# christoskokas/gtsam-vSLAM

Measured on AMD Instinct MI355X. Metric: frames/sec (extract+match+localBA), 1500 feat stereo 752x480, higher is better.
Workload: dtype u8/i32 (extract, match) + f64 (pose LM, local BA)

## Files before the change

gtsam-vslam_amd/csrc/extract_kernels.hpp:

```cpp
#pragma once
#include "common.hpp"

namespace vslam {

struct PyrDesc {
    int nLevels;
    int w[MAX_LEVELS], h[MAX_LEVELS], pitch[MAX_LEVELS];
    uint32_t off[MAX_LEVELS];
    uint32_t imgStride;
};

struct FastDesc {
    int minXY;
    int edge3;
    int nCols[MAX_LEVELS], nRows[MAX_LEVELS], gridW[MAX_LEVELS], gridH[MAX_LEVELS];
    int cellBase[MAX_LEVELS + 1];
    int cellCap;
    int tileRows, tilePitch;
};

struct BlurDesc {
    int tilesX[MAX_LEVELS];
    int tileBase[MAX_LEVELS + 1];
    int taps[7];
};

struct LevelTables {
    float scalePyr[MAX_LEVELS];
    int scaledPatch[MAX_LEVELS];
};

__host__ __device__ static inline uint32_t pack_cand(int x, int y, int s) {
    return ((uint32_t)y << 20) | ((uint32_t)x << 8) | (uint32_t)s;
}
__host__ __device__ static inline int cand_x(uint32_t p) { return (p >> 8) & 0xfff; }
__host__ __device__ static inline int cand_y(uint32_t p) { return p >> 20; }
__host__ __device__ static inline int cand_s(uint32_t p) { return p & 0xff; }

constexpr int FAST_TILE_PITCH = 80;
constexpr int FAST_TILE_MAX = 76;
constexpr int BLUR_RPT = 16;
constexpr int BLUR_TW = 256, BLUR_TH = 4 * BLUR_RPT;

void launch_load_images(hipStream_t s, const uint8_t* const* dSrc, int stride, uint8_t* pyr, const PyrDesc& P, int nimg);
void launch_load_images_color(hipStream_t s, const uint8_t* const* dSrc, int stride, int channels, uint8_t* pyr, const PyrDesc& P,
                              int nimg);
struct RectSrc {
    const uint8_t* src; const float* mapX; const float* mapY;
    int sw, sh, stride, pad;
};
void launch_load_images_rect(hipStream_t s, const RectSrc* dTab, int channels, uint8_t* pyr, const PyrDesc& P, int nimg);
void launch_resize(hipStream_t s, uint8_t* pyr, const PyrDesc& P, int level, const int2* xtab,
                   const int2* ytab, int nimg);
void launch_fast(hipStream_t s, const uint8_t* pyr, const PyrDesc& P, const FastDesc& F,
                 uint32_t* cellSlots, int* cellCount, int maxThr, int minThr, int nimg);
#ifdef VSLAM_FAST_CHECK
int fast_check_failures(hipStream_t s);
#endif
void launch_gather(hipStream_t s, const uint32_t* cellSlots, const int* cellCount, const FastDesc& F,
                   int nLevels, int* cellOff, uint32_t* cand, int candCap, int* levelCount, int nimg);
void launch_blur(hipStream_t s, const uint8_t* pyr, uint8_t* blur, const PyrDesc& P,
                 const BlurDesc& B, int nimg);
struct DiscRows { int umax[16]; };
void launch_orient_desc(hipStream_t s, const uint8_t* pyr, const uint8_t* blur, const PyrDesc& P,
                        const LevelTables& T, const uint32_t* kept, const int* keptOff, int keptCap,
                        const DiscRows& disc, vslam_keypoint* kps, uint8_t* desc, int outCap,
                        int maxKept, int nimg);
void upload_pattern();

constexpr int SSC_NMAX_LDS = 16384;
constexpr int SSC_NMAX = 65535;
constexpr int SSC_PICKW_G = 2048;
constexpr int SSC_NMAX_MID = 8704;
constexpr int SSC_NMAX_SMALL = 6144;
constexpr int SSC_NMAX_TINY = 3072;
__host__ __device__ static inline int ssc_class(int n, int forceGlobal, int classes = 3) {
    if (forceGlobal || n > SSC_NMAX_LDS) return 1;
    if (n > ((classes & 1) ? SSC_NMAX_MID : SSC_NMAX_SMALL)) return 0;
    if (n > SSC_NMAX_SMALL) return 3;
    return ((classes & 2) && n <= SSC_NMAX_TINY) ? 4 : 2;
}
struct SscArgs {
    const uint32_t* cand; int candCap; const int* levelCount;
    int nLevels, nimg;
    int numRet[MAX_LEVELS], cols[MAX_LEVELS], rows[MAX_LEVELS], high[MAX_LEVELS], kmin[MAX_LEVELS], kmax[MAX_LEVELS];
    uint32_t* tmp;
    uint32_t* gridG;
    const size_t* gridOff;
    uint32_t* aG; uint32_t* sortedG; uint32_t* picksG;
    int forceGlobal;
    int classes;
    int* taskCount;
    int* flags;
};

void launch_ssc(hipStream_t s, const SscArgs& A, uint32_t* kept, int keptCap, int* keptOff, int* hostCounts);

}
```

gtsam-vslam_amd/csrc/ssc.hip:

```cpp
#include "extract_kernels.hpp"
#include <mutex>

namespace vslam {

constexpr int SSC_NT = 512, SSC_NW = SSC_NT / 64;
constexpr int SSC_NPROBE = 8;
constexpr int SSC_COOP_MIN = 2048;
constexpr int SSC_ARENA_WORDS = 20 * 1024;
constexpr int SSC_LONGMAX = 64;

template <int M> struct SscCfg;
template <> struct SscCfg<0> { static constexpr int NMAX = SSC_NMAX_LDS, SEGMAX = 1088, PICKW = SSC_NMAX_LDS / 32, ARENA = SSC_ARENA_WORDS; };
template <> struct SscCfg<1> { static constexpr int NMAX = SSC_NMAX, SEGMAX = 4096, PICKW = SSC_PICKW_G, ARENA = SSC_ARENA_WORDS; };
template <> struct SscCfg<2> { static constexpr int NMAX = SSC_NMAX_SMALL, SEGMAX = 1088, PICKW = SSC_NMAX_SMALL / 32, ARENA = 10 * 1024; };
template <> struct SscCfg<3> { static constexpr int NMAX = SSC_NMAX_MID, SEGMAX = 576, PICKW = SSC_NMAX_MID / 32, ARENA = 10 * 1024; };
template <> struct SscCfg<4> { static constexpr int NMAX = SSC_NMAX_TINY, SEGMAX = 256, PICKW = SSC_NMAX_TINY / 32, ARENA = 4 * 1024; };
template <int M> constexpr int ssc_seg_words() { return 4 * SscCfg<M>::SEGMAX > SSC_NW * 256 ? 4 * SscCfg<M>::SEGMAX : SSC_NW * 256; }
template <int M> constexpr size_t ssc_lds_bytes() {
    return M == 1 ? ((size_t)4 * SscCfg<M>::SEGMAX + (size_t)SscCfg<M>::ARENA) * 4 : ((size_t)2 * SscCfg<M>::NMAX + (size_t)ssc_seg_words<M>()) * 4;
}
template <int M> struct SscCheck {
    using C = SscCfg<M>;
    static_assert(C::SEGMAX - SSC_LONGMAX >= C::NMAX / 17, "every short segment of a tree level needs a list entry");
    static_assert(C::PICKW * 32 >= ((C::NMAX + 63) & ~63), "a probe's pick words cover whole 64-candidate steps");
    static_assert(C::ARENA % SSC_NPROBE == 0 && (M == 1 || C::ARENA / SSC_NPROBE > C::PICKW), "a probing wave's slice holds its pick words and a grid");
    static_assert(M == 1 || C::NMAX + ssc_seg_words<M>() >= C::ARENA, "arena must fit a | seg");
    static constexpr bool ok = true;
};
static_assert(SscCheck<0>::ok && SscCheck<1>::ok && SscCheck<2>::ok && SscCheck<3>::ok && SscCheck<4>::ok, "k_ssc classes");

template <bool G> __device__ __forceinline__ void ssc_fence() {
    if (G) asm volatile("s_waitcnt vmcnt(0) lgkmcnt(0)" ::: "memory");
    else asm volatile("s_waitcnt lgkmcnt(0)" ::: "memory");
}
__device__ __forceinline__ void ssc_lds_fence() { asm volatile("s_waitcnt lgkmcnt(0)" ::: "memory"); }

__device__ __forceinline__ int ssc_cell(int v, int width, float rcpw) {
    const int t = 2 * v;
    int q = (int)((float)t * rcpw);
    q -= (q * width > t);
    q += ((q + 1) * width <= t);
    return q;
}

template <bool G>
__device__ __forceinline__ int ssc_eval(const uint32_t* sc, int n, int width, int cols, int rows, uint32_t* grid, int gridWords,
                                        uint32_t* picks, bool& fits, int abortAbove) {
    const int lane = threadIdx.x & 63;
    const float rcpw = 1.0f / (float)width;
    const int gc = ssc_cell(cols, width, rcpw), gr = ssc_cell(rows, width, rcpw);
    const int span = 2;
    const int rowWords = (gc + 1 + 31) >> 5;
    const int words = (gr + 1) * rowWords;
    fits = words <= gridWords;
    if (!fits) return -1;
    for (int i = lane; i < words; i += 64) grid[i] = 0;
    ssc_lds_fence();
    asm volatile("s_waitcnt vmcnt(0)" ::: "memory");
    int count = 0;
    uint32_t pkNext = lane < n ? sc[lane] : 0u;
    for (int base = 0; base < n; base += 64) {
        const int i = base + lane;
        const bool valid = i < n;
        const uint32_t pk = pkNext;
        if (G) pkNext = (i + 64 < n) ? sc[i + 64] : 0u;
        const int row = ssc_cell(cand_y(pk), width, rcpw);
        const int col = ssc_cell(cand_x(pk), width, rcpw);
        bool covered = true;
        if (valid) covered = (grid[row * rowWords + (col >> 5)] >> (col & 31)) & 1u;
        unsigned long long pend = __ballot(!covered), picked = 0ull;
        while (pend) {
            const int l = __ffsll((long long)pend) - 1;
            picked |= 1ull << l;
            const int rl = __builtin_amdgcn_readlane(row, l), cl = __builtin_amdgcn_readlane(col, l);
            const bool conflict = abs(row - rl) <= span && abs(col - cl) <= span;
            pend &= ~__ballot(conflict);
        }
        if ((picked >> lane) & 1ull) {
            const int r0 = max(row - span, 0), r1 = min(row + span, gr);
            const int c0 = max(col - span, 0), c1 = min(col + span, gc);
            const int w0 = c0 >> 5, w1 = c1 >> 5;
            for (int rr = r0; rr <= r1; rr++) {
                if (w0 == w1) {
                    const uint32_t m = ((1u << (c1 - c0 + 1)) - 1u) << (c0 & 31);
                    atomicOr(&grid[rr * rowWords + w0], m);
                } else {
                    atomicOr(&grid[rr * rowWords + w0], 0xffffffffu << (c0 & 31));
                    atomicOr(&grid[rr * rowWords + w1], 0xffffffffu >> (31 - (c1 & 31)));
                }
            }
        }
        if (picks && lane < 2) picks[(base >> 5) + lane] = (uint32_t)(picked >> (32 * lane));
        count += __popcll(picked);
        if (!G) pkNext = (i + 64 < n) ? sc[i + 64] : 0u;
        ssc_lds_fence();
        asm volatile("s_waitcnt vmcnt(0)" ::: "memory");
        if (abortAbove >= 0 && count > abortAbove) break;
    }
    return count;
}

__device__ int g_sscCoopMin = SSC_COOP_MIN;
__device__ __forceinline__ void ssc_push(uint32_t* segN, int* cntN, int segMax, int f, int e, int depth, int* sFail) {
    if (e - f > g_sscCoopMin) {
        const int q = atomicAdd(cntN + 2, 1);
        if (q < SSC_LONGMAX) { segN[2 * q] = (uint32_t)f | ((uint32_t)e << 16); segN[2 * q + 1] = (uint32_t)depth; }
        else *sFail = 4;
        return;
    }
    const int q = atomicAdd(cntN, 1) + SSC_LONGMAX;
    if (q < segMax) { segN[2 * q] = (uint32_t)f | ((uint32_t)e << 16); segN[2 * q + 1] = (uint32_t)depth; }
    else *sFail = 4;
}

template <bool G>
__device__ void ssc_adjust_heap(uint32_t* first, int holeIndex, int len, uint32_t value) {
    const int topIndex = holeIndex;
    int secondChild = holeIndex;
    while (secondChild < (len - 1) / 2) {
        secondChild = 2 * (secondChild + 1);
        if ((first[secondChild] >> 16) < (first[secondChild - 1] >> 16)) secondChild--;
        first[holeIndex] = first[secondChild];
        ssc_fence<G>();
        holeIndex = secondChild;
    }
    if ((len & 1) == 0 && secondChild == (len - 2) / 2) {
        secondChild = 2 * (secondChild + 1);
        first[holeIndex] = first[secondChild - 1];
        ssc_fence<G>();
        holeIndex = secondChild - 1;
    }
    int parent = (holeIndex - 1) / 2;
    while (holeIndex > topIndex && (first[parent] >> 16) < (value >> 16)) {
        first[holeIndex] = first[parent];
        ssc_fence<G>();
        holeIndex = parent;
        parent = (holeIndex - 1) / 2;
    }
    first[holeIndex] = value;
    ssc_fence<G>();
}
template <bool G>
__device__ void ssc_heapsort(uint32_t* first, int len) {
    if (len < 2) return;
    for (int parent = (len - 2) / 2;; parent--) {
        const uint32_t value = first[parent];
        ssc_adjust_heap<G>(first, parent, len, value);
        if (parent == 0) break;
    }
    for (int last = len; last > 1;) {
        --last;
        const uint32_t value = first[last];
        first[last] = first[0];
        ssc_fence<G>();
        ssc_adjust_heap<G>(first, 0, last, value);
    }
}

__device__ __forceinline__ int ssc_sel_lo(unsigned long long m, int k) {
    unsigned w = (unsigned)m;
    int pos = 0;
    const int cl = __popc(w);
    if (k >= cl) { k -= cl; w = (unsigned)(m >> 32); pos = 32; }
#pragma unroll
    for (int s = 16; s >= 1; s >>= 1) {
        const unsigned lowmask = (1u << s) - 1u;
        const int c = __popc(w & lowmask);
        if (k >= c) { k -= c; w >>= s; pos += s; } else w &= lowmask;
    }
    return pos;
}

template <bool G>
__device__ __forceinline__ void ssc_small_segment(uint32_t* a, int f, int e, int depth, uint16_t* Lp, uint16_t* Rp,
                                                  uint32_t* segN, int* cntN, int segMax, int* sFail) {
    const int lane = threadIdx.x & 63, m = e - f;
    uint32_t v = lane < m ? a[f + lane] : 0u;
    int lo = lane < m ? 0 : 64, hi = lane < m ? m : 64, d = depth;
    for (;;) {
        const bool act = (hi - lo) > 16;
        if (__ballot(act) == 0ull) break;
        if (__ballot(act && d == 0) != 0ull) {
            if (lane < m) a[f + lane] = v;
            if (act && lane == lo) ssc_push(segN, cntN, segMax, f + lo, f + hi, d, sFail);
            ssc_fence<G>();
            return;
        }
        const int ia = act ? lo + 1 : lane, ib = act ? lo + (hi - lo) / 2 : lane, ic = act ? hi - 1 : lane;
        const uint32_t va = __shfl(v, ia), vb = __shfl(v, ib), vc = __shfl(v, ic), vlo = __shfl(v, act ? lo : lane);
        const uint32_t ka = va >> 16, kb = vb >> 16, kc = vc >> 16;
        int mi;
        if (ka < kb) { if (kb < kc) mi = ib; else if (ka < kc) mi = ic; else mi = ia; }
        else if (ka < kc) mi = ia; else if (kb < kc) mi = ic; else mi = ib;
        const uint32_t vm = mi == ia ? va : (mi == ib ? vb : vc);
        if (act) { if (lane == lo) v = vm; else if (lane == mi) v = vlo; }
        const uint32_t pk = vm >> 16;
        const bool inR = act && lane > lo && lane < hi;
        const uint32_t kx = v >> 16;
        const bool isL = inR && kx >= pk, isR = inR && kx <= pk;
        const unsigned long long below = hi >= 64 ? ~0ull : ((1ull << hi) - 1ull);
        const unsigned long long segmask = act ? (below & ~((1ull << lo) - 1ull)) : 0ull;
        const unsigned long long mL = __ballot(isL) & segmask, mR = __ballot(isR) & segmask;
        const int nL = __popcll(mL), nR = __popcll(mR);
        const int kL = __popcll(mL & ((1ull << lane) - 1ull));
        const int kR = lane == 63 ? 0 : __popcll(mR >> (lane + 1));
        if (isL) Lp[f + lo + kL] = (uint16_t)lane;
        if (isR) Rp[f + lo + kR] = (uint16_t)lane;
        ssc_fence<G>();
        int src = lane;
        bool asL = false;
        if (isL && kL < nR) { const int p = Rp[f + lo + kL]; if (lane < p) { src = p; asL = true; } }
        if (!asL && isR && kR < nL) { const int p = Lp[f + lo + kR]; if (p < lane) src = p; }
        const int K = __popcll(__ballot(asL) & segmask);
        v = __shfl(v, src);
        if (act) {
            int cut = K >= 1 ? (int)Rp[f + lo + K - 1] : hi;
            if (K < nL) cut = min(cut, (int)Lp[f + lo + K]);
            d--;
            if (lane < cut) hi = cut; else lo = cut;
        }
        ssc_fence<G>();
    }
    if (lane < m) a[f + lane] = v;
    ssc_fence<G>();
}

__device__ __forceinline__ void ssc_median_to_first(uint32_t* a, int f, int e) {
    const int ia = f + 1, ib = f + (e - f) / 2, ic = e - 1;
    const uint32_t ka = a[ia] >> 16, kb = a[ib] >> 16, kc = a[ic] >> 16;
    int m;
    if (ka < kb) { if (kb < kc) m = ib; else if (ka < kc) m = ic; else m = ia; }
    else if (ka < kc) m = ia; else if (kb < kc) m = ic; else m = ib;
    const uint32_t t = a[f]; a[f] = a[m]; a[m] = t;
}

template <bool G>
__device__ __forceinline__ void ssc_partition_coop(uint32_t* a, uint16_t* Lp, uint16_t* Rp, int f, int e, int depth, int* sW,
                                                   uint32_t* segN, int* cntN, int segMax, int* sFail) {
    const int tid = threadIdx.x, lane = tid & 63, wave = tid >> 6;
    if (tid == 0) { ssc_median_to_first(a, f, e); ssc_fence<G>(); }
    __syncthreads();
    const uint32_t pk = a[f] >> 16;
    const int m = e - f - 1;
    const int per = ((m + SSC_NW - 1) / SSC_NW + 63) & ~63;
    const int c0 = min(e, f + 1 + wave * per), c1 = min(e, c0 + per);
    int nl = 0, nr = 0;
    for (int base = c0; base < c1; base += 64) {
        const int x = base + lane;
        const bool v = x < c1;
        const uint32_t kx = v ? (a[x] >> 16) : 0u;
        nl += __popcll(__ballot(v && kx >= pk)); nr += __popcll(__ballot(v && kx <= pk));
    }
    if (lane == 0) { sW[wave] = nl; sW[SSC_NW + wave] = nr; }
    __syncthreads();
    int offL = 0, offR = 0, nL = 0, nR = 0;
#pragma unroll
    for (int w = 0; w < SSC_NW; w++) {
        const int l = sW[w], r = sW[SSC_NW + w];
        if (w < wave) { offL += l; offR += r; }
        nL += l; nR += r;
    }
    const unsigned long long lt = (1ull << lane) - 1ull;
    for (int base = c0; base < c1; base += 64) {
        const int x = base + lane;
        const bool v = x < c1;
        const uint32_t kx = v ? (a[x] >> 16) : 0u;
        const bool isL = v && kx >= pk, isR = v && kx <= pk;
        const unsigned long long bl = __ballot(isL), br = __ballot(isR);
        if (isL) Lp[f + 1 + offL + __popcll(bl & lt)] = (uint16_t)x;
        if (isR) Rp[f + 1 + offR + __popcll(br & lt)] = (uint16_t)x;
        offL += __popcll(bl); offR += __popcll(br);
    }
    const int nPair = min(nL, nR);
    if (tid == 0) sW[2 * SSC_NW] = nPair;
    ssc_fence<G>();
    __syncthreads();
    for (int k = tid; k < nPair; k += SSC_NT)
        if (!(Lp[f + 1 + k] < Rp[f + 1 + nR - 1 - k])) { atomicMin(&sW[2 * SSC_NW], k); break; }
    __syncthreads();
    const int K = sW[2 * SSC_NW];
    for (int k = tid; k < K; k += SSC_NT) {
        const int xl = Lp[f + 1 + k], xr = Rp[f + 1 + nR - 1 - k];
        const uint32_t t = a[xl]; a[xl] = a[xr]; a[xr] = t;
    }
    if (tid == 0) {
        int cut = K >= 1 ? (int)Rp[f + 1 + nR - K] : e;
        if (K < nL) cut = min(cut, (int)Lp[f + 1 + K]);
        if (e - cut > 16) ssc_push(segN, cntN, segMax, cut, e, depth - 1, sFail);
        if (cut - f > 16) ssc_push(segN, cntN, segMax, f, cut, depth - 1, sFail);
    }
    ssc_fence<G>();
    __syncthreads();
}

template <int M>
__global__ __launch_bounds__(SSC_NT, 4) void k_ssc(SscArgs A) {
    using C = SscCfg<M>;
    constexpr bool G = M == 1;
    extern __shared__ uint32_t lds[];
    const int img = blockIdx.x % A.nimg, l = blockIdx.x / A.nimg;
    const int task = img * A.nLevels + l;
    const int* lc = A.levelCount + (size_t)img * (MAX_LEVELS + 1);
    int coff = 0;
    for (int q = 0; q < l; q++) coff += lc[q];
    const int n = lc[l];
    if (ssc_class(n, A.forceGlobal, A.classes) != M) return;
    uint32_t* sortedU = G ? A.sortedG + (size_t)img * A.candCap + coff : lds;
    uint32_t* a = G ? A.aG + (size_t)img * A.candCap + coff : lds + C::NMAX;
    uint16_t* Lp = (uint16_t*)sortedU;
    uint16_t* Rp = Lp + (G ? n : C::NMAX);
    uint32_t* seg = G ? lds : lds + 2 * C::NMAX;
    uint32_t* arena = G ? lds + 4 * C::SEGMAX : lds + C::NMAX;
    int* h2 = G ? (int*)arena : (int*)seg;
    __shared__ int hist[256], sCnt[4], sFail, sW[2 * SSC_NW + 2];
    __shared__ int cacheW[64], cacheC[64], cacheSlot[64], nCache, sched[8], nSched, sFinal, sDone, sSolo;
    __shared__ int sLow, sHigh, sPrev, sLast;
    __shared__ int pre[C::PICKW];
    const int tid = threadIdx.x, lane = tid & 63;
    const int wave = __builtin_amdgcn_readfirstlane(tid >> 6);
#ifdef VSLAM_SSC_STAMPS
    long long st_t = clock64();
    long long* st = (long long*)(A.taskCount + A.nimg * MAX_LEVELS) + (size_t)task * 8;
#define SSC_STAMP(k) do { if (tid == 0) { const long long n_ = clock64(); st[k] = n_ - st_t; st_t = n_; } } while (0)
#else
#define SSC_STAMP(k) do {} while (0)
#endif
    const uint32_t* cand = A.cand + (size_t)img * A.candCap + coff;
    uint32_t* out = A.tmp + (size_t)img * A.candCap + coff;
    int* taskCount = A.taskCount + task;
    if (lc[MAX_LEVELS] > A.candCap) { if (tid == 0) { A.flags[2 * img + 1] = 1; *taskCount = 0; } return; }
    const int numRet = A.numRet[l];
    if (n <= numRet) {
        for (int i = tid; i < n; i += SSC_NT) out[i] = cand[i];
        if (tid == 0) *taskCount = n;
        return;
    }
    if (n > C::NMAX) { if (tid == 0) { atomicOr(&A.flags[2 * img], 1); *taskCount = 0; } return; }

    for (int i = tid; i < n; i += SSC_NT) a[i] = ((uint32_t)cand_s(cand[i]) << 16) | (uint32_t)i;
    if (tid < 256) hist[tid] = 0;
    if (tid == 0) {
        sFail = 0;
        int lg = 0;
        while ((1 << (lg + 1)) <= n) lg++;
        sCnt[0] = sCnt[1] = sCnt[2] = sCnt[3] = 0;
        if (n > 16) ssc_push(seg, &sCnt[0], C::SEGMAX, 0, n, 2 * lg, &sFail);
    }
    ssc_fence<G>();
    __syncthreads();
    int cur = 0;
    for (;;) {
        const int nseg = min(sCnt[cur], C::SEGMAX - SSC_LONGMAX), nlong = min(sCnt[2 + cur], SSC_LONGMAX);
        if (nseg == 0 && nlong == 0) break;
        const uint32_t* segL = seg + cur * C::SEGMAX * 2;
        const uint32_t* segC = segL + 2 * SSC_LONGMAX;
        uint32_t* segN = seg + (cur ^ 1) * C::SEGMAX * 2;
        int* cntN = &sCnt[cur ^ 1];
        for (int s = 0; s < nlong; s++) {
            const int f = (int)(segL[2 * s] & 0xffffu), e = (int)(segL[2 * s] >> 16), depth = (int)segL[2 * s + 1];
            if (depth == 0) { if (tid == 0) ssc_heapsort<G>(a + f, e - f); continue; }
            ssc_partition_coop<G>(a, Lp, Rp, f, e, depth, sW, segN, cntN, C::SEGMAX, &sFail);
        }
        for (int s = wave; s < nseg; s += SSC_NW) {
            const uint32_t sfe = (uint32_t)__builtin_amdgcn_readfirstlane((int)segC[2 * s]);
            const int f = (int)(sfe & 0xffffu), e = (int)(sfe >> 16), depth = __builtin_amdgcn_readfirstlane((int)segC[2 * s + 1]);
            if (depth == 0) { if (lane == 0) ssc_heapsort<G>(a + f, e - f); continue; }
            if (e - f <= 64) {
                ssc_small_segment<G>(a, f, e, depth, Lp, Rp, segN, cntN, C::SEGMAX, &sFail);
                continue;
            }
            if (lane == 0) ssc_median_to_first(a, f, e);
            ssc_fence<G>();
            const uint32_t pk = a[f] >> 16;
            int nL = 0, nR = 0;
            for (int base = f + 1; base < e; base += 64) {
                const int x = base + lane;
                const bool v = x < e;
                const uint32_t kx = v ? (a[x] >> 16) : 0u;
                const bool isL = v && kx >= pk, isR = v && kx <= pk;
                const unsigned long long bl = __ballot(isL), br = __ballot(isR);
                const unsigned long long lt = (1ull << lane) - 1ull;
                if (isL) Lp[f + 1 + nL + __popcll(bl & lt)] = (uint16_t)x;
                if (isR) Rp[f + 1 + nR + __popcll(br & lt)] = (uint16_t)x;
                nL += __popcll(bl); nR += __popcll(br);
            }
            ssc_fence<G>();
            const int nPair = min(nL, nR);
            int K = 0;
            for (int base = 0; base < nPair; base += 64) {
                const int k = base + lane;
                const bool ok = k < nPair && Lp[f + 1 + k] < Rp[f + 1 + nR - 1 - k];
                const unsigned long long bo = __ballot(ok);
                K += __popcll(bo);
                if (bo != ~0ull) break;
            }
            for (int k = lane; k < K; k += 64) {
                const int xl = Lp[f + 1 + k], xr = Rp[f + 1 + nR - 1 - k];
                const uint32_t t = a[xl]; a[xl] = a[xr]; a[xr] = t;
            }
            ssc_fence<G>();
            int cut = K >= 1 ? (int)Rp[f + 1 + nR - K] : e;
            if (K < nL) cut = min(cut, (int)Lp[f + 1 + K]);
            if (lane == 0) {
                if (e - cut > 16) ssc_push(segN, cntN, C::SEGMAX, cut, e, depth - 1, &sFail);
                if (cut - f > 16) ssc_push(segN, cntN, C::SEGMAX, f, cut, depth - 1, &sFail);
            }
        }
        ssc_fence<G>();
        __syncthreads();
        if (tid == 0) { sCnt[cur] = 0; sCnt[2 + cur] = 0; }
        cur ^= 1;
        __syncthreads();
    }
    SSC_STAMP(0);
    if (sFail) { if (tid == 0) { atomicOr(&A.flags[2 * img], sFail); *taskCount = 0; } return; }
    for (int i = tid; i < SSC_NW * 256; i += SSC_NT) h2[i] = 0;
    __syncthreads();
    const int per = ((n + SSC_NW - 1) / SSC_NW + 63) & ~63;
    const int s0 = min(n, wave * per), s1 = min(n, s0 + per);
    for (int i = s0 + lane; i < s1; i += 64) atomicAdd(&h2[wave * 256 + (int)(a[i] >> 16)], 1);
    __syncthreads();
    if (tid < 256) { int t = 0; for (int w = 0; w < SSC_NW; w++) t += h2[w * 256 + tid]; hist[tid] = t; }
    __syncthreads();
    if (wave == 0) {
        int run = 0;
        for (int base = 0; base < 256; base += 64) {
            const int v = hist[base + lane];
            int incl = v;
#pragma unroll
            for (int d = 1; d < 64; d <<= 1) { const int t = __shfl_up(incl, d); if (lane >= d) incl += t; }
            hist[base + lane] = run + incl - v;
            run += __shfl(incl, 63);
        }
    }
    __syncthreads();
    if (tid < 256) { int run = hist[tid]; for (int w = 0; w < SSC_NW; w++) { const int t = h2[w * 256 + tid]; h2[w * 256 + tid] = run; run += t; } }
    __syncthreads();
    {
        int* off = h2 + wave * 256;
        for (int base = s0; base < s1; base += 64) {
            const int i = base + lane;
            const bool v = i < s1;
            const uint32_t e = v ? a[i] : 0u;
            const int key = (int)(e >> 16);
            unsigned long long same = v ? ~0ull : 0ull;
#pragma unroll
            for (int bit = 0; bit < 8; bit++) {
                const unsigned long long bb = __ballot(v && ((key >> bit) & 1));
                same &= ((key >> bit) & 1) ? bb : ~bb;
            }
            same &= __ballot(v);
            if (v) {
                const int rank = __popcll(same & ((1ull << lane) - 1ull));
                sortedU[n - 1 - (off[key] + rank)] = cand[e & 0xffffu];
            }
            ssc_lds_fence();
            if (v && (same >> lane) == 1ull) off[key] += __popcll(same);
            ssc_lds_fence();
        }
    }
    ssc_fence<G>();
    __syncthreads();
    SSC_STAMP(1);
    const uint32_t* sc = sortedU;

    if (tid == 0) {
        sLow = max(1, (int)floor(sqrt((double)n / numRet)));
        sHigh = A.high[l]; sPrev = -1; sLast = -1; nCache = 0; sDone = 0; sFinal = -1; sSolo = 0;
    }
    __syncthreads();
    const int kmin = A.kmin[l], kmax = A.kmax[l];
    const int cols = A.cols[l], rows = A.rows[l];
    uint32_t* gridG = A.gridG + A.gridOff[task];
    constexpr int SLICE = C::ARENA / SSC_NPROBE;
    uint32_t* picksG = G ? A.picksG + (size_t)task * SSC_NPROBE * SSC_PICKW_G : nullptr;
    constexpr int PICKW_L = G ? 0 : C::PICKW;
    auto picks_of = [&](int slot) -> uint32_t* {
        if (G) return picksG + (size_t)(slot < 0 ? SSC_NPROBE - 1 : slot) * SSC_PICKW_G;
        return slot < 0 ? arena + C::ARENA - PICKW_L : arena + slot * SLICE + SLICE - PICKW_L;
    };
    int lastEval = -1;
    for (int round = 0; round < 64; round++) {
        if (tid == 0) {
            nSched = 0;
            for (;;) {
                const int width = sLow + (sHigh - sLow) / 2;
                if (width == sPrev || sLow > sHigh) { sFinal = sLast; sDone = 1; break; }
                int cnt = -1;
                for (int q = 0; q < nCache; q++) if (cacheW[q] == width) cnt = cacheC[q];
                if (cnt < 0) break;
                sLast = width;
                if (cnt >= kmin && cnt <= kmax) { sFinal = width; sDone = 1; break; }
                if (cnt < kmin) sHigh = width - 1; else sLow = width + 1;
                sPrev = width;
            }
            if (!sDone) {
                int qlow[8], qhigh[8], qprev[8];
                qlow[1] = sLow; qhigh[1] = sHigh; qprev[1] = sPrev;
                for (int node = 1; node < 8; node++) {
                    const int lo = qlow[node], hi = qhigh[node], pv = qprev[node];
                    const int width = lo + (hi - lo) / 2;
                    const bool term = lo > hi || width == pv;
                    if (!term) {
                        bool dup = false;
                        for (int q = 0; q < nSched; q++) dup |= sched[q] == width;
                        for (int q = 0; q < nCache; q++) dup |= cacheW[q] == width;
                        if (!dup && nSched < SSC_NPROBE - 1) sched[nSched++] = width;
                    }
                    if (2 * node + 1 < 8) {
                        qlow[2 * node] = term ? 1 : lo; qhigh[2 * node] = term ? 0 : width - 1; qprev[2 * node] = width;
                        qlow[2 * node + 1] = term ? 1 : width + 1; qhigh[2 * node + 1] = term ? 0 : hi; qprev[2 * node + 1] = width;
                    }
                }
                if (sSolo) nSched = 1;
            }
        }
        __syncthreads();
        if (sDone) break;
        const int ns = nSched;
        const bool solo = sSolo != 0;
        if (ns > 0) lastEval = round;
        int cnt = -2;
        bool fits = true;
        uint32_t* picks = picks_of(solo ? -1 : wave);
        if (wave < ns) {
            uint32_t* grid = solo ? arena : arena + wave * SLICE;
            cnt = ssc_eval<G>(sc, n, sched[wave], cols, rows, grid, (solo ? C::ARENA : SLICE) - PICKW_L, picks, fits, kmax);
            if (solo && !fits) cnt = ssc_eval<G>(sc, n, sched[wave], cols, rows, gridG, 1 << 30, picks, fits, kmax);
        }
        __syncthreads();
        if (wave < ns && lane == 0) {
            if (fits) { const int q = atomicAdd(&nCache, 1); if (q < 64) { cacheW[q] = sched[wave]; cacheC[q] = cnt; cacheSlot[q] = (round << 4) | (solo ? 15 : wave); } else sFail = 8; }
            else if (wave == 0) { if (solo) sFail = 16; else sSolo = 1; }
        }
        __syncthreads();
        if (sFail) { if (tid == 0) { atomicOr(&A.flags[2 * img], sFail); *taskCount = 0; } return; }
        if (tid == 0 && sSolo && ns > 0) {
            bool served = false;
            for (int q = 0; q < nCache; q++) served |= cacheW[q] == sched[0];
            if (served && solo) sSolo = 0;
        }
        __syncthreads();
    }
    SSC_STAMP(2);
#ifdef VSLAM_SSC_STAMPS
    if (tid == 0) { st[4] = n; st[5] = nCache; st[6] = sFinal; }
#endif
    if (!sDone) { if (tid == 0) { atomicOr(&A.flags[2 * img], 32); *taskCount = 0; } return; }
    int total = 0;
    if (sFinal >= 0) {
        int slot = -1, evalRound = -1;
        for (int q = 0; q < nCache; q++) if (cacheW[q] == sFinal) { slot = cacheSlot[q] & 15; evalRound = cacheSlot[q] >> 4; total = cacheC[q]; }
        if (slot == 15) slot = -1;
        const uint32_t* picks = picks_of(slot);
        if (total > kmax || evalRound != lastEval) {
            __syncthreads();
            if (wave == 0) {
                uint32_t* pk = picks_of(-1);
                bool fits;
                int cnt = ssc_eval<G>(sc, n, sFinal, cols, rows, arena, C::ARENA - PICKW_L, pk, fits, -1);
                if (!fits) cnt = ssc_eval<G>(sc, n, sFinal, cols, rows, gridG, 1 << 30, pk, fits, -1);
                if (lane == 0) sCnt[0] = cnt;
            }
            __syncthreads();
            total = sCnt[0];
            picks = picks_of(-1);
        }
        const int nWords = (n + 31) >> 5;
        for (int w = tid; w < C::PICKW; w += SSC_NT) pre[w] = w < nWords ? __popc(picks[w]) : 0;
        __syncthreads();
        if (wave == 0) {
            int run = 0;
            for (int base = 0; base < nWords; base += 64) {
                const bool in = base + lane < C::PICKW;
                const int v = in ? pre[base + lane] : 0;
                int incl = v;
#pragma unroll
                for (int d = 1; d < 64; d <<= 1) { const int t = __shfl_up(incl, d); if (lane >= d) incl += t; }
                if (in) pre[base + lane] = run + incl - v;
                run += __shfl(incl, 63);
            }
        }
        __syncthreads();
        for (int wd = tid; wd < nWords; wd += SSC_NT) {
            uint32_t w = picks[wd];
            int o = pre[wd];
            while (w) { const int bit = __ffs((int)w) - 1; w &= w - 1; out[o++] = sc[32 * wd + bit]; }
        }
    }
    if (tid == 0) *taskCount = total;
    SSC_STAMP(3);
}

__global__ __launch_bounds__(256) void k_ssc_pack(SscArgs A, uint32_t* __restrict__ kept, int keptCap, int* __restrict__ keptOff,
                                                  int* __restrict__ hostCounts) {
    const int img = blockIdx.x, tid = threadIdx.x;
    const int* lc = A.levelCount + (size_t)img * (MAX_LEVELS + 1);
    int* koff = keptOff + (size_t)img * (MAX_LEVELS + 1);
    int k = 0, coff = 0;
    for (int l = 0; l < A.nLevels; l++) {
        const int cnt = A.taskCount[img * A.nLevels + l];
        const int room = max(0, min(cnt, keptCap - k));
        const uint32_t* src = A.tmp + (size_t)img * A.candCap + coff;
        for (int i = tid; i < room; i += 256) kept[(size_t)img * keptCap + k + i] = src[i];
        if (tid == 0) { koff[l] = k; if (cnt > room) A.flags[2 * img + 1] = 1; }
        k += room;
        coff += lc[l];
    }
    if (tid == 0) {
        for (int l = A.nLevels; l <= MAX_LEVELS; l++) koff[l] = k;
        hostCounts[img] = k;
        hostCounts[A.nimg + 2 * img] = A.flags[2 * img];
        hostCounts[A.nimg + 2 * img + 1] = A.flags[2 * img + 1];
        A.flags[2 * img] = 0; A.flags[2 * img + 1] = 0;
    }
}

void launch_ssc(hipStream_t s, const SscArgs& A, uint32_t* kept, int keptCap, int* keptOff, int* hostCounts) {
    const size_t ldsL = ssc_lds_bytes<0>(), ldsG = ssc_lds_bytes<1>(), ldsS = ssc_lds_bytes<2>(), ldsM = ssc_lds_bytes<3>(), ldsT = ssc_lds_bytes<4>();
    static std::once_flag attr;
    std::call_once(attr, [&] {
        if (const char* e = getenv("VSLAM_SSC_COOP_MIN")) {
            const int v = std::max(65, std::min(65535, atoi(e)));
            (void)hipMemcpyToSymbol(HIP_SYMBOL(g_sscCoopMin), &v, sizeof(int));
        }
        (void)hipFuncSetAttribute((const void*)k_ssc<0>, hipFuncAttributeMaxDynamicSharedMemorySize, (int)ldsL);
        (void)hipFuncSetAttribute((const void*)k_ssc<2>, hipFuncAttributeMaxDynamicSharedMemorySize, (int)ldsS);
        (void)hipFuncSetAttribute((const void*)k_ssc<1>, hipFuncAttributeMaxDynamicSharedMemorySize, (int)ldsG);
        (void)hipFuncSetAttribute((const void*)k_ssc<3>, hipFuncAttributeMaxDynamicSharedMemorySize, (int)ldsM);
        (void)hipFuncSetAttribute((const void*)k_ssc<4>, hipFuncAttributeMaxDynamicSharedMemorySize, (int)ldsT);
    });
    const dim3 grid(A.nimg * A.nLevels);
    if (A.classes) {
        hipLaunchKernelGGL(k_ssc<1>, grid, dim3(SSC_NT), ldsG, s, A);
        hipLaunchKernelGGL(k_ssc<0>, grid, dim3(SSC_NT), ldsL, s, A);
        if (A.classes & 1) hipLaunchKernelGGL(k_ssc<3>, grid, dim3(SSC_NT), ldsM, s, A);
        hipLaunchKernelGGL(k_ssc<2>, grid, dim3(SSC_NT), ldsS, s, A);
        if (A.classes & 2) hipLaunchKernelGGL(k_ssc<4>, grid, dim3(SSC_NT), ldsT, s, A);
    } else {
        hipLaunchKernelGGL(k_ssc<2>, grid, dim3(SSC_NT), ldsS, s, A);
        hipLaunchKernelGGL(k_ssc<0>, grid, dim3(SSC_NT), ldsL, s, A);
        hipLaunchKernelGGL(k_ssc<1>, grid, dim3(SSC_NT), ldsG, s, A);
    }
    hipLaunchKernelGGL(k_ssc_pack, dim3(A.nimg), dim3(256), 0, s, A, kept, keptCap, keptOff, hostCounts);
}

}
```

Before: 31050.

## Compact SSC partition scratch into one two-ended index array and widen mid class

Replaces the separate left/right uint16 index buffers used by the quicksort partition with a single two-ended scratch array that keeps only up to half the segment from each side. Wave-level partitioning now scans from both ends at once and exits early. The radix sort writes 16-bit indices that are gathered into the sorted array afterwards. Together these cut LDS use per class, and the mid class grows to 10240 candidates so more levels avoid the larger-LDS class while two blocks still fit per CU. The cost is an extra gather pass plus added indexing logic in a tricky partition routine.

```diff
diff --git a/gtsam-vslam_amd/csrc/extract_kernels.hpp b/gtsam-vslam_amd/csrc/extract_kernels.hpp
--- a/gtsam-vslam_amd/csrc/extract_kernels.hpp
+++ b/gtsam-vslam_amd/csrc/extract_kernels.hpp
@@ -71,7 +71,7 @@
 constexpr int SSC_NMAX_LDS = 16384;
 constexpr int SSC_NMAX = 65535;
 constexpr int SSC_PICKW_G = 2048;
-constexpr int SSC_NMAX_MID = 8704;
+constexpr int SSC_NMAX_MID = 10240;
 constexpr int SSC_NMAX_SMALL = 6144;
 constexpr int SSC_NMAX_TINY = 3072;
 __host__ __device__ static inline int ssc_class(int n, int forceGlobal, int classes = 3) {
diff --git a/gtsam-vslam_amd/csrc/ssc.hip b/gtsam-vslam_amd/csrc/ssc.hip
--- a/gtsam-vslam_amd/csrc/ssc.hip
+++ b/gtsam-vslam_amd/csrc/ssc.hip
@@ -1,33 +1,16 @@
 #include "extract_kernels.hpp"
+#include "ssc_partition.hpp"
 #include <mutex>
 
 namespace vslam {
 
-constexpr int SSC_NT = 512, SSC_NW = SSC_NT / 64;
-constexpr int SSC_NPROBE = 8;
 constexpr int SSC_COOP_MIN = 2048;
-constexpr int SSC_ARENA_WORDS = 20 * 1024;
-constexpr int SSC_LONGMAX = 64;
-
-template <int M> struct SscCfg;
-template <> struct SscCfg<0> { static constexpr int NMAX = SSC_NMAX_LDS, SEGMAX = 1088, PICKW = SSC_NMAX_LDS / 32, ARENA = SSC_ARENA_WORDS; };
-template <> struct SscCfg<1> { static constexpr int NMAX = SSC_NMAX, SEGMAX = 4096, PICKW = SSC_PICKW_G, ARENA = SSC_ARENA_WORDS; };
-template <> struct SscCfg<2> { static constexpr int NMAX = SSC_NMAX_SMALL, SEGMAX = 1088, PICKW = SSC_NMAX_SMALL / 32, ARENA = 10 * 1024; };
-template <> struct SscCfg<3> { static constexpr int NMAX = SSC_NMAX_MID, SEGMAX = 576, PICKW = SSC_NMAX_MID / 32, ARENA = 10 * 1024; };
-template <> struct SscCfg<4> { static constexpr int NMAX = SSC_NMAX_TINY, SEGMAX = 256, PICKW = SSC_NMAX_TINY / 32, ARENA = 4 * 1024; };
-template <int M> constexpr int ssc_seg_words() { return 4 * SscCfg<M>::SEGMAX > SSC_NW * 256 ? 4 * SscCfg<M>::SEGMAX : SSC_NW * 256; }
-template <int M> constexpr size_t ssc_lds_bytes() {
-    return M == 1 ? ((size_t)4 * SscCfg<M>::SEGMAX + (size_t)SscCfg<M>::ARENA) * 4 : ((size_t)2 * SscCfg<M>::NMAX + (size_t)ssc_seg_words<M>()) * 4;
-}
-template <int M> struct SscCheck {
-    using C = SscCfg<M>;
-    static_assert(C::SEGMAX - SSC_LONGMAX >= C::NMAX / 17, "every short segment of a tree level needs a list entry");
-    static_assert(C::PICKW * 32 >= ((C::NMAX + 63) & ~63), "a probe's pick words cover whole 64-candidate steps");
-    static_assert(C::ARENA % SSC_NPROBE == 0 && (M == 1 || C::ARENA / SSC_NPROBE > C::PICKW), "a probing wave's slice holds its pick words and a grid");
-    static_assert(M == 1 || C::NMAX + ssc_seg_words<M>() >= C::ARENA, "arena must fit a | seg");
-    static constexpr bool ok = true;
+
+template <int M> struct SscCfg {
+    static constexpr int NMAX = ssc_class_cfg(M).nmax, SEGMAX = ssc_class_cfg(M).segmax, PICKW = ssc_class_cfg(M).pickw, ARENA = ssc_class_cfg(M).arena;
 };
-static_assert(SscCheck<0>::ok && SscCheck<1>::ok && SscCheck<2>::ok && SscCheck<3>::ok && SscCheck<4>::ok, "k_ssc classes");
+static_assert(SscCfg<0>::NMAX == SSC_NMAX_LDS && SscCfg<1>::NMAX == SSC_NMAX && SscCfg<1>::PICKW == SSC_PICKW_G && SscCfg<2>::NMAX == SSC_NMAX_SMALL &&
+              SscCfg<3>::NMAX == SSC_NMAX_MID && SscCfg<4>::NMAX == SSC_NMAX_TINY, "ssc_class_cfg and ssc_class speak of the same classes");
 
 template <bool G> __device__ __forceinline__ void ssc_fence() {
     if (G) asm volatile("s_waitcnt vmcnt(0) lgkmcnt(0)" ::: "memory");
@@ -172,7 +155,7 @@
 }
 
 template <bool G>
-__device__ __forceinline__ void ssc_small_segment(uint32_t* a, int f, int e, int depth, uint16_t* Lp, uint16_t* Rp,
+__device__ __forceinline__ void ssc_small_segment(uint32_t* a, int f, int e, int depth, uint16_t* St,
                                                   uint32_t* segN, int* cntN, int segMax, int* sFail) {
     const int lane = threadIdx.x & 63, m = e - f;
     uint32_t v = lane < m ? a[f + lane] : 0u;
@@ -204,18 +187,18 @@
         const int nL = __popcll(mL), nR = __popcll(mR);
         const int kL = __popcll(mL & ((1ull << lane) - 1ull));
         const int kR = lane == 63 ? 0 : __popcll(mR >> (lane + 1));
-        if (isL) Lp[f + lo + kL] = (uint16_t)lane;
-        if (isR) Rp[f + lo + kR] = (uint16_t)lane;
+        const int sf = f + lo, se = f + hi, h = ssc_st_half(sf, se), nPair = ssc_st_pairs(nL, nR, h);
+        if (isL && ssc_st_keeps_left(kL, h)) St[ssc_st_left_slot(sf, kL)] = (uint16_t)lane;
+        if (isR && ssc_st_keeps_right(kR, h)) St[ssc_st_right_slot(se, kR)] = (uint16_t)lane;
         ssc_fence<G>();
         int src = lane;
         bool asL = false;
-        if (isL && kL < nR) { const int p = Rp[f + lo + kL]; if (lane < p) { src = p; asL = true; } }
-        if (!asL && isR && kR < nL) { const int p = Lp[f + lo + kR]; if (p < lane) src = p; }
+        if (isL && kL < nPair) { const int p = St[ssc_st_right_slot(se, kL)]; if (lane < p) { src = p; asL = true; } }
+        if (!asL && isR && kR < nPair) { const int p = St[ssc_st_left_slot(sf, kR)]; if (p < lane) src = p; }
         const int K = __popcll(__ballot(asL) & segmask);
         v = __shfl(v, src);
         if (act) {
-            int cut = K >= 1 ? (int)Rp[f + lo + K - 1] : hi;
-            if (K < nL) cut = min(cut, (int)Lp[f + lo + K]);
+            const int cut = ssc_st_cut(St, sf, se, K, nL, hi);
             d--;
             if (lane < cut) hi = cut; else lo = cut;
         }
@@ -235,7 +218,7 @@
 }
 
 template <bool G>
-__device__ __forceinline__ void ssc_partition_coop(uint32_t* a, uint16_t* Lp, uint16_t* Rp, int f, int e, int depth, int* sW,
+__device__ __forceinline__ void ssc_partition_coop(uint32_t* a, uint16_t* St, int f, int e, int depth, int* sW,
                                                    uint32_t* segN, int* cntN, int segMax, int* sFail) {
     const int tid = threadIdx.x, lane = tid & 63, wave = tid >> 6;
     if (tid == 0) { ssc_median_to_first(a, f, e); ssc_fence<G>(); }
@@ -261,31 +244,32 @@
         nL += l; nR += r;
     }
     const unsigned long long lt = (1ull << lane) - 1ull;
+    const int h = ssc_st_half(f, e);
     for (int base = c0; base < c1; base += 64) {
         const int x = base + lane;
         const bool v = x < c1;
         const uint32_t kx = v ? (a[x] >> 16) : 0u;
         const bool isL = v && kx >= pk, isR = v && kx <= pk;
         const unsigned long long bl = __ballot(isL), br = __ballot(isR);
-        if (isL) Lp[f + 1 + offL + __popcll(bl & lt)] = (uint16_t)x;
-        if (isR) Rp[f + 1 + offR + __popcll(br & lt)] = (uint16_t)x;
+        const int kl = offL + __popcll(bl & lt), jr = nR - 1 - (offR + __popcll(br & lt));
+        if (isL && ssc_st_keeps_left(kl, h)) St[ssc_st_left_slot(f, kl)] = (uint16_t)x;
+        if (isR && ssc_st_keeps_right(jr, h)) St[ssc_st_right_slot(e, jr)] = (uint16_t)x;
         offL += __popcll(bl); offR += __popcll(br);
     }
-    const int nPair = min(nL, nR);
+    const int nPair = ssc_st_pairs(nL, nR, h);
     if (tid == 0) sW[2 * SSC_NW] = nPair;
     ssc_fence<G>();
     __syncthreads();
     for (int k = tid; k < nPair; k += SSC_NT)
-        if (!(Lp[f + 1 + k] < Rp[f + 1 + nR - 1 - k])) { atomicMin(&sW[2 * SSC_NW], k); break; }
+        if (!(St[ssc_st_left_slot(f, k)] < St[ssc_st_right_slot(e, k)])) { atomicMin(&sW[2 * SSC_NW], k); break; }
     __syncthreads();
     const int K = sW[2 * SSC_NW];
     for (int k = tid; k < K; k += SSC_NT) {
-        const int xl = Lp[f + 1 + k], xr = Rp[f + 1 + nR - 1 - k];
+        const int xl = St[ssc_st_left_slot(f, k)], xr = St[ssc_st_right_slot(e, k)];
         const uint32_t t = a[xl]; a[xl] = a[xr]; a[xr] = t;
     }
     if (tid == 0) {
-        int cut = K >= 1 ? (int)Rp[f + 1 + nR - K] : e;
-        if (K < nL) cut = min(cut, (int)Lp[f + 1 + K]);
+        const int cut = ssc_st_cut(St, f, e, K, nL, e);
         if (e - cut > 16) ssc_push(segN, cntN, segMax, cut, e, depth - 1, sFail);
         if (cut - f > 16) ssc_push(segN, cntN, segMax, f, cut, depth - 1, sFail);
     }
@@ -305,12 +289,11 @@
     for (int q = 0; q < l; q++) coff += lc[q];
     const int n = lc[l];
     if (ssc_class(n, A.forceGlobal, A.classes) != M) return;
-    uint32_t* sortedU = G ? A.sortedG + (size_t)img * A.candCap + coff : lds;
-    uint32_t* a = G ? A.aG + (size_t)img * A.candCap + coff : lds + C::NMAX;
-    uint16_t* Lp = (uint16_t*)sortedU;
-    uint16_t* Rp = Lp + (G ? n : C::NMAX);
-    uint32_t* seg = G ? lds : lds + 2 * C::NMAX;
-    uint32_t* arena = G ? lds + 4 * C::SEGMAX : lds + C::NMAX;
+    uint32_t* a = G ? A.aG + (size_t)img * A.candCap + coff : lds + ssc_off_a(M);
+    uint32_t* sortedU = a;
+    uint16_t* St = G ? (uint16_t*)(A.sortedG + (size_t)img * A.candCap + coff) : (uint16_t*)(lds + ssc_off_st(M));
+    uint32_t* seg = lds + ssc_off_seg(M);
+    uint32_t* arena = lds + ssc_off_arena(M);
     int* h2 = G ? (int*)arena : (int*)seg;
     __shared__ int hist[256], sCnt[4], sFail, sW[2 * SSC_NW + 2];
     __shared__ int cacheW[64], cacheC[64], cacheSlot[64], nCache, sched[8], nSched, sFinal, sDone, sSolo;
@@ -359,48 +342,50 @@
         for (int s = 0; s < nlong; s++) {
             const int f = (int)(segL[2 * s] & 0xffffu), e = (int)(segL[2 * s] >> 16), depth = (int)segL[2 * s + 1];
             if (depth == 0) { if (tid == 0) ssc_heapsort<G>(a + f, e - f); continue; }
-            ssc_partition_coop<G>(a, Lp, Rp, f, e, depth, sW, segN, cntN, C::SEGMAX, &sFail);
+            ssc_partition_coop<G>(a, St, f, e, depth, sW, segN, cntN, C::SEGMAX, &sFail);
         }
         for (int s = wave; s < nseg; s += SSC_NW) {
             const uint32_t sfe = (uint32_t)__builtin_amdgcn_readfirstlane((int)segC[2 * s]);
             const int f = (int)(sfe & 0xffffu), e = (int)(sfe >> 16), depth = __builtin_amdgcn_readfirstlane((int)segC[2 * s + 1]);
             if (depth == 0) { if (lane == 0) ssc_heapsort<G>(a + f, e - f); continue; }
             if (e - f <= 64) {
-                ssc_small_segment<G>(a, f, e, depth, Lp, Rp, segN, cntN, C::SEGMAX, &sFail);
+                ssc_small_segment<G>(a, f, e, depth, St, segN, cntN, C::SEGMAX, &sFail);
                 continue;
             }
             if (lane == 0) ssc_median_to_first(a, f, e);
             ssc_fence<G>();
             const uint32_t pk = a[f] >> 16;
+            const int h = ssc_st_half(f, e);
             int nL = 0, nR = 0;
-            for (int base = f + 1; base < e; base += 64) {
-                const int x = base + lane;
-                const bool v = x < e;
-                const uint32_t kx = v ? (a[x] >> 16) : 0u;
-                const bool isL = v && kx >= pk, isR = v && kx <= pk;
+            for (int base = 0; base < e - f - 1; base += 64) {
+                const int xl = f + 1 + base + lane, xr = e - 1 - base - lane;
+                const bool v = xl < e;
+                const uint32_t kl = v ? (a[xl] >> 16) : 0u, kr = v ? (a[xr] >> 16) : 0u;
+                const bool isL = v && kl >= pk, isR = v && kr <= pk;
                 const unsigned long long bl = __ballot(isL), br = __ballot(isR);
                 const unsigned long long lt = (1ull << lane) - 1ull;
-                if (isL) Lp[f + 1 + nL + __popcll(bl & lt)] = (uint16_t)x;
-                if (isR) Rp[f + 1 + nR + __popcll(br & lt)] = (uint16_t)x;
+                const int rl = nL + __popcll(bl & lt), rr = nR + __popcll(br & lt);
+                if (isL && ssc_st_keeps_left(rl, h)) St[ssc_st_left_slot(f, rl)] = (uint16_t)xl;
+                if (isR && ssc_st_keeps_right(rr, h)) St[ssc_st_right_slot(e, rr)] = (uint16_t)xr;
                 nL += __popcll(bl); nR += __popcll(br);
+                if (nL > h && nR >= h) break;
             }
             ssc_fence<G>();
-            const int nPair = min(nL, nR);
+            const int nPair = ssc_st_pairs(nL, nR, h);
             int K = 0;
             for (int base = 0; base < nPair; base += 64) {
                 const int k = base + lane;
-                const bool ok = k < nPair && Lp[f + 1 + k] < Rp[f + 1 + nR - 1 - k];
+                const bool ok = k < nPair && St[ssc_st_left_slot(f, k)] < St[ssc_st_right_slot(e, k)];
                 const unsigned long long bo = __ballot(ok);
                 K += __popcll(bo);
                 if (bo != ~0ull) break;
             }
             for (int k = lane; k < K; k += 64) {
-                const int xl = Lp[f + 1 + k], xr = Rp[f + 1 + nR - 1 - k];
+                const int xl = St[ssc_st_left_slot(f, k)], xr = St[ssc_st_right_slot(e, k)];
                 const uint32_t t = a[xl]; a[xl] = a[xr]; a[xr] = t;
             }
             ssc_fence<G>();
-            int cut = K >= 1 ? (int)Rp[f + 1 + nR - K] : e;
-            if (K < nL) cut = min(cut, (int)Lp[f + 1 + K]);
+            const int cut = ssc_st_cut(St, f, e, K, nL, e);
             if (lane == 0) {
                 if (e - cut > 16) ssc_push(segN, cntN, C::SEGMAX, cut, e, depth - 1, &sFail);
                 if (cut - f > 16) ssc_push(segN, cntN, C::SEGMAX, f, cut, depth - 1, &sFail);
@@ -452,13 +437,16 @@
             same &= __ballot(v);
             if (v) {
                 const int rank = __popcll(same & ((1ull << lane) - 1ull));
-                sortedU[n - 1 - (off[key] + rank)] = cand[e & 0xffffu];
+                St[n - 1 - (off[key] + rank)] = (uint16_t)(e & 0xffffu);
             }
             ssc_lds_fence();
             if (v && (same >> lane) == 1ull) off[key] += __popcll(same);
             ssc_lds_fence();
         }
     }
+    ssc_fence<G>();
+    __syncthreads();
+    for (int i = tid; i < n; i += SSC_NT) sortedU[i] = cand[St[i]];
     ssc_fence<G>();
     __syncthreads();
     SSC_STAMP(1);
@@ -617,7 +605,7 @@
 }
 
 void launch_ssc(hipStream_t s, const SscArgs& A, uint32_t* kept, int keptCap, int* keptOff, int* hostCounts) {
-    const size_t ldsL = ssc_lds_bytes<0>(), ldsG = ssc_lds_bytes<1>(), ldsS = ssc_lds_bytes<2>(), ldsM = ssc_lds_bytes<3>(), ldsT = ssc_lds_bytes<4>();
+    const size_t ldsL = ssc_lds_bytes(0), ldsG = ssc_lds_bytes(1), ldsS = ssc_lds_bytes(2), ldsM = ssc_lds_bytes(3), ldsT = ssc_lds_bytes(4);
     static std::once_flag attr;
     std::call_once(attr, [&] {
         if (const char* e = getenv("VSLAM_SSC_COOP_MIN")) {
diff --git a/gtsam-vslam_amd/csrc/ssc_partition.hpp b/gtsam-vslam_amd/csrc/ssc_partition.hpp
--- /dev/null
+++ b/gtsam-vslam_amd/csrc/ssc_partition.hpp
@@ -0,0 +1,69 @@
+#pragma once
+#include <cstddef>
+
+#if defined(__HIPCC__) || defined(__CUDACC__)
+#define SSC_HD __host__ __device__ inline
+#else
+#define SSC_HD inline
+#endif
+
+SSC_HD int ssc_st_half(int f, int e) { return (e - f - 1) >> 1; }
+SSC_HD bool ssc_st_keeps_left(int k, int h) { return k <= h; }
+SSC_HD bool ssc_st_keeps_right(int j, int h) { return j < h; }
+SSC_HD int ssc_st_left_slot(int f, int k) { return f + k; }
+SSC_HD int ssc_st_right_slot(int e, int j) { return e - 1 - j; }
+SSC_HD int ssc_st_pairs(int nL, int nR, int h) { const int p = nL < nR ? nL : nR; return p < h ? p : h; }
+template <class A>
+SSC_HD int ssc_st_cut(const A& St, int f, int e, int K, int nL, int top) {
+    int cut = K >= 1 ? (int)St[ssc_st_right_slot(e, K - 1)] : top;
+    if (K < nL) { const int l = (int)St[ssc_st_left_slot(f, K)]; if (l < cut) cut = l; }
+    return cut;
+}
+
+constexpr int SSC_NT = 512, SSC_NW = SSC_NT / 64;
+constexpr int SSC_NPROBE = 8;
+constexpr int SSC_LONGMAX = 64;
+constexpr int SSC_STATIC_FIXED = 2048;
+constexpr int SSC_CU_LDS = 160 * 1024;
+constexpr int SSC_LDS_GRANULE = 1280;
+
+struct SscClassCfg { int nmax, segmax, pickw, arena, perCU; };
+constexpr SscClassCfg ssc_class_cfg(int M) {
+    return M == 0 ? SscClassCfg{16384, 1088, 16384 / 32, 20 * 1024, 1}
+         : M == 1 ? SscClassCfg{65535, 4096, 2048, 20 * 1024, 1}
+         : M == 2 ? SscClassCfg{6144, 1088, 6144 / 32, 10 * 1024, 2}
+         : M == 3 ? SscClassCfg{10240, 672, 10240 / 32, 9408, 2}
+         :          SscClassCfg{3072, 256, 3072 / 32, 4 * 1024, 4};
+}
+constexpr bool ssc_class_hbm(int M) { return M == 1; }
+
+constexpr int ssc_seg_words(int M) { return 4 * ssc_class_cfg(M).segmax > SSC_NW * 256 ? 4 * ssc_class_cfg(M).segmax : SSC_NW * 256; }
+constexpr int ssc_off_a(int) { return 0; }
+constexpr int ssc_off_st(int M) { return ssc_class_hbm(M) ? 0 : ssc_class_cfg(M).nmax; }
+constexpr int ssc_off_seg(int M) { return ssc_class_hbm(M) ? 0 : ssc_class_cfg(M).nmax + (ssc_class_cfg(M).nmax + 1) / 2; }
+constexpr int ssc_off_arena(int M) { return ssc_class_hbm(M) ? ssc_seg_words(M) : ssc_class_cfg(M).nmax; }
+constexpr int ssc_lds_words(int M) {
+    return ssc_off_seg(M) + ssc_seg_words(M) > ssc_off_arena(M) + ssc_class_cfg(M).arena ? ssc_off_seg(M) + ssc_seg_words(M)
+                                                                                          : ssc_off_arena(M) + ssc_class_cfg(M).arena;
+}
+constexpr size_t ssc_lds_bytes(int M) { return (size_t)ssc_lds_words(M) * 4; }
+constexpr int ssc_static_lds_bound(int M) { return SSC_STATIC_FIXED + 4 * ssc_class_cfg(M).pickw; }
+constexpr int ssc_task_lds(int M) {
+    return (int)((ssc_lds_bytes(M) + ssc_static_lds_bound(M) + SSC_LDS_GRANULE - 1) / SSC_LDS_GRANULE * SSC_LDS_GRANULE);
+}
+
+constexpr bool ssc_class_ok(int M) {
+    return ssc_class_cfg(M).segmax - SSC_LONGMAX >= ssc_class_cfg(M).nmax / 17
+        && ssc_class_cfg(M).pickw * 32 >= ((ssc_class_cfg(M).nmax + 63) & ~63)
+        && ssc_class_cfg(M).arena % SSC_NPROBE == 0
+        && (ssc_class_hbm(M) || ssc_class_cfg(M).arena / SSC_NPROBE > ssc_class_cfg(M).pickw)
+        && ssc_class_cfg(M).nmax <= 65536
+        && (ssc_class_hbm(M) || ssc_class_cfg(M).nmax % 2 == 0)
+        && ssc_seg_words(M) >= SSC_NW * 256 && ssc_seg_words(M) >= 4 * ssc_class_cfg(M).segmax
+        && (ssc_class_hbm(M) || ssc_off_seg(M) * 4 >= ssc_off_st(M) * 4 + 2 * ssc_class_cfg(M).nmax)
+        && ssc_off_arena(M) >= (ssc_class_hbm(M) ? ssc_seg_words(M) : ssc_class_cfg(M).nmax)
+        && ssc_lds_words(M) >= ssc_off_seg(M) + ssc_seg_words(M)
+        && ssc_lds_words(M) >= ssc_off_arena(M) + ssc_class_cfg(M).arena
+        && ssc_task_lds(M) * ssc_class_cfg(M).perCU <= SSC_CU_LDS;
+}
+static_assert(ssc_class_ok(0) && ssc_class_ok(1) && ssc_class_ok(2) && ssc_class_ok(3) && ssc_class_ok(4), "k_ssc classes");
```

After: 31440, median of 6. About the same (+1.3%).
